# cv3vpl-lab/cylinder-pose-estimation

Hardware: AMD Instinct MI355X
Metric: frames/sec (grid-detect + cylinder fit) on 1920x1200 batch (higher is better)
Workload: dtype f64

## Files before the change

cylinder-pose-estimation_amd/csrc/ccl.hip:

```cpp
#include "cpe_dev.h"

namespace cpe {

namespace {

__device__ __forceinline__ bool pred(const uint8_t *img, size_t i, int thr, int invert)
{
    return (((int)img[i] > thr) ? 1 : 0) != invert;
}

constexpr int CCL_INIT_ROWS = 16;
__global__ __launch_bounds__(256) void k_ccl_init(const uint8_t *__restrict__ img, int rows_total, int h, int w,
                                                  int thr, int invert, const FrameState *__restrict__ st, Window win,
                                                  int *__restrict__ L, int *__restrict__ cnt, CclOutside outside)
{
    const int lane = threadIdx.x & 63;
    for (int rr = 0; rr < CCL_INIT_ROWS / 4; rr++) {
    const int row = (blockIdx.x * (CCL_INIT_ROWS / 4) + rr) * 4 + (threadIdx.x >> 6);
    if (row >= rows_total) return;
    const int f = row / h, y = row - f * h;
    const Rect r = window_rect(st, f, win, h, w);
    if (y < r.y0 || y > r.y1 || r.x1 < r.x0) continue;
    const size_t base = (size_t)row * w;
    int carry_in = 0, carry_start = 0;
// ... 876 lines not shown
static bool links8(const uint8_t *img, int n, int h, int w, int thr, Window win, int *L, FrameState *st, hipStream_t s)
{
    const size_t N = (size_t)h * w;
    if (word_rows(img, L, w)) {
        const ByteSrc src{img, w, thr, 0};
        CPE_KLAUNCH(k_ccl_init64<ByteSrc>, word_grid(n, h, w), dim3(256), 0, s, src, h, w, (const FrameState *)st, win, L);
        CPE_KLAUNCH(k_ccl_merge64<ByteSrc>, word_grid(n, h, w), dim3(256), 0, s, src, h, w, 1, (const FrameState *)st, win, L);
        return true;
    }
    CPE_KLAUNCH(k_ccl_init, dim3((n * h + CCL_INIT_ROWS - 1) / CCL_INIT_ROWS), dim3(256), 0, s, img, n * h, h, w, thr, 0, (const FrameState *)st, win, L,
                (int *)nullptr, OUTSIDE_UNTOUCHED);
    CPE_KLAUNCH(k_ccl_merge, dim3((unsigned)((N + CCL_BLK_PX - 1) / CCL_BLK_PX), n), dim3(256), 0, s, img, h, w, thr, 0, 1, (const FrameState *)st, win, L);
    return false;
}

int ccl_components(const uint8_t *img, const uint32_t *bits, int n, int h, int w, int thr, Window win, int *L, int *roots,
                   RootList list, FrameState *st, hipStream_t s)
{
    const size_t N = (size_t)h * w;
    const dim3 gw = word_grid(n, h, w);
    CPE_LAUNCH_BEGIN();
    CPE_KLAUNCH(k_ccl_ctl, dim3((n + 63) / 64), dim3(64), 0, s, st, (int *)nullptr, n, CTL_RESET_ROOTS, list);
    if (bits && w % 16 == 0 && ((size_t)L & 15) == 0) {
        const BitSrc src{bit_plane(bits, 0, h, w), bit_tile_cols(w), bit_plane_words(h, w)};
        CPE_KLAUNCH(k_ccl_init64<BitSrc>, gw, dim3(256), 0, s, src, h, w, (const FrameState *)st, win, L);
        CPE_KLAUNCH(k_ccl_merge64<BitSrc>, gw, dim3(256), 0, s, src, h, w, 1, (const FrameState *)st, win, L);
        CPE_KLAUNCH(k_ccl_roots64<BitSrc>, gw, dim3(256), 0, s, src, h, w, st, win, (const int *)L, roots, list);
    } else if (links8(img, n, h, w, thr, win, L, st, s)) {
        CPE_KLAUNCH(k_ccl_roots64<ByteSrc>, gw, dim3(256), 0, s, (ByteSrc{img, w, thr, 0}), h, w, st, win, (const int *)L, roots, list);
    } else {
        CPE_KLAUNCH(k_ccl_roots4, dim3((unsigned)((N + CCL_BLK_PX - 1) / CCL_BLK_PX), n), dim3(256), 0, s, img, h, w, thr, 0, st, win, (const int *)L,
                    roots, list);
    }
    CPE_CHECK_LAUNCH("ccl_components");
    return CPE_OK;
}

int ccl_unions(const uint8_t *mask, int n, int h, int w, Window win, int *L, FrameState *st, hipStream_t s)
// ... 61 lines not shown
```

cylinder-pose-estimation_amd/csrc/cpe_dev.h:

```cpp
#pragma once
#include "cpe_internal.h"

namespace cpe {

constexpr int MAXROOTS = 262144;
enum { SWL_DARK = 0, SWL_BRIGHT = 1, SWL_TRACE = 2 };
__host__ __device__ inline int sweep_pool(int h, int w, int which)
{
    const long long N = (long long)h * w;
    long long v = which == SWL_TRACE ? N / 8 : N / 2;
    const long long lo = which == SWL_TRACE ? (1 << 18) : (1 << 19);
    v = v < lo ? lo : (v > (1 << 23) ? (1 << 23) : v);
    return (int)((v + 255) / 256 * 256);
}
constexpr int MAXJ = CPE_MAXJ;
constexpr int MAXB = 32768;
constexpr int MAXG = 32768;
constexpr int MAXG_LDS = 1024;
constexpr int GCAP = 48;
constexpr int MAXV = 131072;
constexpr int MAXL = CPE_MAXL;
constexpr int MAXLP = CPE_MAXLP;
constexpr int MAXSEG = 2048;

// ... 50 lines not shown
    int *lohi, *hull;
};
struct RegionProbe {
    int identity;
    double *blobs; int blob_cap; int *n_blobs;
    float *kp; int kp_cap; int *n_kp;
};
inline unsigned frame_waves(int lists, int lo, int hi)
{
    const int v = 16384 / (lists > 0 ? lists : 1);
    return (unsigned)(v < lo ? lo : (v > hi ? hi : v));
}
struct RegionSide { hipStream_t s; hipEvent_t clahe_done, dark_done, traced, medians;
                    hipEvent_t joints_done = nullptr, spot_done = nullptr; };
struct MaskBuffers {
    uint8_t *binary, *hmask, *vmask, *joints_mask, *tmpA, *tmpB, *g19, *cm, *mc, *roi_h, *roi_v, *base_h, *base_v, *exp_h,
        *exp_v, *touch;
    int *lab, *roots, *jtmp, *joints, *verts;
    int *lab_p, *roots_p, *lab_s, *roots_s;
    int *lab_h, *lab_v;
    uint32_t *bits;
    unsigned long long *best, *best_s;
    unsigned long long *fl_j;
    uint32_t *jbits;
    SegRec *segs;
};

enum { OVF_ROOTS = 1, OVF_LINES = 2, OVF_TRACE = 4, OVF_JOINTS = 8, OVF_VERTS = 16, OVF_SEGS = 32, OVF_KERNEL = 64,
       OVF_EXPAND = 128, OVF_BLOBS = 256, OVF_DISTS = 512, OVF_GROUPS = 1024, OVF_SWEEP = 2048 };
__device__ __forceinline__ void set_overflow(FrameState &S, int bit) { atomicOr(&S.overflow, bit); }

// ... 226 lines not shown
    double d00 = (double)a00;
    if (fabs(d00) > 1.1920928955078125e-07) {
        double db1_2, db1_6;
        if (d00 > 0) { db1_2 = 0.5; db1_6 = 0.16666666666666666666666666666667; }
        else { db1_2 = -0.5; db1_6 = -0.16666666666666666666666666666667; }
        m00 = d00 * db1_2;
        m10 = (double)a10 * db1_6;
        m01 = (double)a01 * db1_6;
    }
}

int build_bitplanes(const uint8_t *img, int n, int h, int w, int thr0, int step, int nplanes, uint32_t *planes, hipStream_t s);

int ccl_components(const uint8_t *img, const uint32_t *bits, int n, int h, int w, int thr, Window win, int *L, int *roots,
                   RootList list, FrameState *st, hipStream_t s);
int ccl_unions(const uint8_t *mask, int n, int h, int w, Window win, int *L, FrameState *st, hipStream_t s);
int ccl_dark_first(const uint8_t *img, const uint32_t *planes, int nplanes, int n, int h, int w, int thr, int *L, int *roots,
                   int *cnt, FrameState *st, hipStream_t s);
enum CclOutside : int { OUTSIDE_NONE = 0, OUTSIDE_UNTOUCHED = 1, OUTSIDE_SWEEP_RUNS = 3 };
enum CclCount : int { COUNT_NONE = 0, COUNT_ALL = 1, COUNT_INTERIOR = 2, COUNT_ZERO = 3 };
struct CclPass {
    int thr = 0, invert = 0, conn8 = 1;
    Window win = WIN_FRAME;
    CclOutside outside = OUTSIDE_NONE;
    CclCount count = COUNT_NONE; int *cnt = nullptr;
    uint8_t *touch = nullptr;
    int *roots = nullptr;
    int *nrect = nullptr;
};
int ccl_label(const uint8_t *img, int n, int h, int w, int *L, const CclPass &p, FrameState *st, hipStream_t s);
// ... 29 lines not shown
```

cylinder-pose-estimation_amd/csrc/detect.hip:

```cpp
#include "workspace.h"
#include <ctype.h>
#include <mutex>
#include <stdlib.h>

namespace cpe {

namespace {

__global__ void k_state_init(FrameState *st, int n, unsigned long long *best, unsigned long long *best_s, int *nrect)
{
    int f = blockIdx.x * blockDim.x + threadIdx.x;
    if (f >= n) return;
    FrameState z = {};
    z.srect[0] = INT_MAX; z.srect[1] = INT_MAX; z.srect[2] = -1; z.srect[3] = -1;
    st[f] = z;
    if (best) { best[f] = 0; best_s[f] = 0; }
    if (nrect) { nrect[16 * f] = INT_MAX; nrect[16 * f + 1] = INT_MAX; nrect[16 * f + 2] = -1; nrect[16 * f + 3] = -1; }
}

__global__ void k_finish(const FrameState *st, int n, int *status, int *n_pts)
{
    int f = blockIdx.x * blockDim.x + threadIdx.x;
    if (f >= n) return;
    int s = st[f].status;
// ... 53 lines not shown
    R.lab = W.at<int>(WS_LABELS); R.cnt = W.at<int>(WS_LABELS_AUX); R.roots = W.at<int>(WS_ROOTS); R.nrect = W.at<int>(WS_NRECT);
    R.lab2 = W.at<int>(WS_BRIGHT_NODES); R.cnt2 = W.at<int>(WS_BRIGHT_COUNTS); R.sw = W.at<int>(WS_SWEEP); R.bk = W.at<int>(WS_BUCKET_PIXELS);
    R.hl = W.at<int2>(WS_LIST_DARK); R.bl = W.at<int2>(WS_LIST_BRIGHT); R.tl = W.at<int2>(WS_LIST_TRACE);
    R.bits = W.at<uint32_t>(WS_BITS); R.pool = W.at<uint32_t>(WS_POOL); R.blob_ch = W.at<unsigned short>(WS_BLOB_CH);
    R.maxch = region_maxch(h, w); R.maxdf = region_maxdf(h, w); R.gmid = W.at<double>(WS_GMID);
    R.hist = W.at<unsigned int>(WS_HIST); R.lut = W.at<uint8_t>(WS_LUT);
    R.blobs = W.at<BlobRec>(WS_BLOBS); R.blob_d = W.at<int>(WS_BLOB_D); R.order = W.at<int>(WS_ORDER); R.dists = W.at<double>(WS_DISTS);
    R.groups = W.at<Group>(WS_GROUPS); R.best = W.at<unsigned long long>(WS_BEST); R.lohi = W.at<int>(WS_LOHI); R.hull = W.at<int>(WS_HULL);
    return R;
}

MaskBuffers mask_buffers(const Workspace &W, const RegionBuffers &R)
{
    MaskBuffers M;
    M.binary = W.at<uint8_t>(WS_BINARY); M.hmask = W.at<uint8_t>(WS_HMASK); M.vmask = W.at<uint8_t>(WS_VMASK);
    M.joints_mask = W.at<uint8_t>(WS_JOINTS_MASK); M.tmpA = W.at<uint8_t>(WS_TMPA); M.tmpB = W.at<uint8_t>(WS_TMPB);
    M.g19 = W.at<uint8_t>(WS_BLUR19); M.cm = W.at<uint8_t>(WS_CM); M.mc = R.mc; M.roi_h = W.at<uint8_t>(WS_ROI_H);
    M.roi_v = W.at<uint8_t>(WS_ROI_V); M.base_h = W.at<uint8_t>(WS_BASE_H); M.base_v = W.at<uint8_t>(WS_BASE_V);
    M.exp_h = W.at<uint8_t>(WS_EXP_H); M.exp_v = W.at<uint8_t>(WS_EXP_V); M.touch = R.touch; M.bits = R.bits;
    M.lab = R.lab; M.roots = R.roots; M.jtmp = W.at<int>(WS_JTMP); M.joints = W.at<int>(WS_JOINTS); M.verts = W.at<int>(WS_VERTS);
    M.best = R.best; M.segs = W.at<SegRec>(WS_SEGS);
    M.lab_p = W.at<int>(WS_LABELS_JOINTS); M.lab_s = W.at<int>(WS_LABELS_SPOT);
    M.roots_p = W.at<int>(WS_ROOTS_JOINTS); M.roots_s = W.at<int>(WS_ROOTS_SPOT); M.best_s = W.at<unsigned long long>(WS_BEST_SPOT);
    M.fl_j = W.at<unsigned long long>(WS_FLJ); M.jbits = W.at<uint32_t>(WS_JOINT_BITS);
    M.lab_h = nullptr; M.lab_v = nullptr;
    return M;
}

}
}

// ... 460 lines not shown
```

cylinder-pose-estimation_amd/csrc/masks.hip:

```cpp
#include "cpe_dev.h"

namespace cpe {

namespace {

struct W3 { unsigned long long a, b, c; };
template <int K> __device__ __forceinline__ W3 w3_up(const W3 &v, unsigned long long fill)
{
    W3 r;
    r.a = (v.a >> K) | (v.b << (64 - K));
    r.b = (v.b >> K) | (v.c << (64 - K));
    r.c = (v.c >> K) | (fill << (64 - K));
    return r;
}
template <int K> __device__ __forceinline__ W3 w3_down(const W3 &v, unsigned long long fill)
{
    W3 r;
    r.c = (v.c << K) | (v.b >> (64 - K));
    r.b = (v.b << K) | (v.a >> (64 - K));
    r.a = (v.a << K) | (fill >> (64 - K));
    return r;
}
__device__ __forceinline__ W3 w3_and(const W3 &x, const W3 &y) { return W3{x.a & y.a, x.b & y.b, x.c & y.c}; }
__device__ __forceinline__ W3 w3_or(const W3 &x, const W3 &y) { return W3{x.a | y.a, x.b | y.b, x.c | y.c}; }
// ... 126 lines not shown
                    hm[o + b] = ((hb >> b) & 1u) ? 255 : 0;
                    vm[o + b] = ((vb >> b) & 1u) ? 255 : 0;
                    jm[o + b] = (((hb & vb) >> b) & 1u) ? 255 : 0;
                }
            }
        }
        store_plane_band(bit_plane(jbits, f, h, w), h, w, y0, R, t, [&](int tr, int j) {
            const size_t wi = (size_t)tr * WW + j;
            unsigned long long m = hbuf[wi] & (buf0[wi] | ((tr + 12 < ROWS) ? buf1[wi + (size_t)12 * WW] : 0ull));
            if (64 * j + 64 > w) m &= (1ull << (w - 64 * j)) - 1ull;
            return m;
        });
    }
}

__global__ __launch_bounds__(256) void k_or_and(const uint8_t *__restrict__ a, const uint8_t *__restrict__ b,
                                                const uint8_t *__restrict__ c, int h, int w, const FrameState *__restrict__ st,
                                                uint8_t *__restrict__ dst)
{
    const int N = h * w;
    const size_t f = blockIdx.y;
    const int *r = st[f].rect;
    const bool none = st[f].status == CPE_ST_NO_REGION;
    const int y0 = r[1], y1 = r[1] + r[3] - 1;
    const size_t o = f * (size_t)N;
    const bool vec = ((((size_t)a | (size_t)b | (size_t)c | (size_t)dst) & 15) == 0) && (N % 16 == 0);
    for (int it = 0; it < 4; it++) {
        const int i0 = blockIdx.x * 16384 + it * 4096 + threadIdx.x * 16;
        if (i0 >= N) break;
        const int ya = i0 / w, yb = min(i0 + 15, N - 1) / w;
        const bool outside = none || yb < y0 || ya > y1;
        if (vec) {
            uint4 v = make_uint4(0, 0, 0, 0);
            if (!outside) {
                const uint4 va = *reinterpret_cast<const uint4 *>(a + o + i0), vb = *reinterpret_cast<const uint4 *>(b + o + i0);
                const uint4 vc = *reinterpret_cast<const uint4 *>(c + o + i0);
                auto f4 = [](uint32_t x, uint32_t y, uint32_t z) {
                    uint32_t r4 = 0;
#pragma unroll
                    for (int k = 0; k < 4; k++) {
                        const uint32_t on = (((x | y) >> (8 * k)) & 255u) ? 255u : 0u;
                        r4 |= (on & ((z >> (8 * k)) & 255u)) << (8 * k);
                    }
                    return r4;
                };
                v = make_uint4(f4(va.x, vb.x, vc.x), f4(va.y, vb.y, vc.y), f4(va.z, vb.z, vc.z), f4(va.w, vb.w, vc.w));
            }
            *reinterpret_cast<uint4 *>(dst + o + i0) = v;
        } else {
            for (int k = 0; k < 16 && i0 + k < N; k++) {
                const size_t gi = o + i0 + k;
                dst[gi] = outside ? 0 : (uint8_t)(((a[gi] ? 255 : 0) | (b[gi] ? 255 : 0)) & c[gi]);
            }
        }
    }
}

constexpr int RB_R = 64, RB_AP = 4, RB_ROWS = RB_R + 2 * RB_AP;
__global__ __launch_bounds__(256) void k_roi_base(const uint8_t *__restrict__ m, const uint8_t *__restrict__ cm,
                                                  const uint8_t *__restrict__ mc, int h, int w, int bands,
                                                  const FrameState *__restrict__ st, uint8_t *__restrict__ roi,
                                                  uint8_t *__restrict__ base, uint32_t *__restrict__ bbits)
{
    extern __shared__ unsigned long long s_rb[];
    const int WW = (w + 63) >> 6;
    unsigned long long *buf0 = s_rb, *buf1 = s_rb + (size_t)RB_ROWS * WW;
    const int t = threadIdx.x;
    const int f = blockIdx.x / bands, band = blockIdx.x - f * bands;
    const int y0 = band * RB_R;
    const size_t N = (size_t)h * w;
    const int *rc = st[f].rect;
    const int rx0 = rc[0], ry0 = rc[1], rx1 = rc[0] + rc[2] - 1, ry1 = rc[1] + rc[3] - 1;
    const bool al8 = ((w & 7) == 0) && ((((size_t)m | (size_t)cm | (size_t)mc | (size_t)roi | (size_t)base) & 7) == 0);
    const int per_row = WW * 8;
    auto store8 = [&](uint8_t *dst, size_t o, int x0, unsigned bits) {
        if (al8) *reinterpret_cast<unsigned long long *>(dst + o) = bytes_of_bits8(bits);
        else for (int b = 0; b < 8 && x0 + b < w; b++) dst[o + b] = ((bits >> b) & 1u) ? 255 : 0;
    };
    if (st[f].status == CPE_ST_NO_REGION || y0 > ry1 + RB_AP || y0 + RB_R - 1 < ry0 - RB_AP) {
        for (int i = t; i < RB_R * per_row; i += 256) {
            const int tr = i / per_row, k = i - tr * per_row;
            const int y = y0 + tr, x0 = k * 8;
            if (y >= h || x0 >= w) continue;
            const size_t o = f * N + (size_t)y * w + x0;
            store8(roi, o, x0, 0u); store8(base, o, x0, 0u);
        }
        store_plane_band(bit_plane(bbits, f, h, w), h, w, y0, RB_R, t, [](int, int) { return 0ull; });
        return;
    }
    {
        uint8_t *pk = reinterpret_cast<uint8_t *>(buf0);
        for (int i = t; i < RB_ROWS * per_row; i += 256) {
            const int r = i / per_row, k = i - r * per_row;
            const int y = y0 - RB_AP + r, x0 = k * 8;
            unsigned bits = 0u;
            if (y >= ry0 && y <= ry1 && y >= 0 && y < h && x0 < w && x0 + 7 >= rx0 && x0 <= rx1) {
                const size_t o = f * N + (size_t)y * w + x0;
                if (al8) {
                    unsigned long long v = *reinterpret_cast<const unsigned long long *>(m + o) &
                                           *reinterpret_cast<const unsigned long long *>(cm + o) &
                                           *reinterpret_cast<const unsigned long long *>(mc + o);
                    v = (((v & 0x7f7f7f7f7f7f7f7full) + 0x7f7f7f7f7f7f7f7full) | v) & 0x8080808080808080ull;
                    bits = (unsigned)(((v >> 7) * 0x0102040810204080ull) >> 56);
                } else {
                    for (int b = 0; b < 8 && x0 + b < w; b++) bits |= ((m[o + b] & cm[o + b]) & mc[o + b]) ? (1u << b) : 0u;
                }
            }
            pk[i] = (uint8_t)bits;
        }
    }
    __syncthreads();
    auto pass = [&](const unsigned long long *src, unsigned long long *dst, bool dil) {
        const unsigned long long fill = dil ? 0ull : ~0ull;
        for (int i = t; i < RB_ROWS * WW; i += 256) {
            const int r = i / WW, j = i - r * WW;
            unsigned long long acc = fill;
#pragma unroll
            for (int dr = -1; dr <= 1; dr++) {
                const int rr = r + dr, y = y0 - RB_AP + rr;
                unsigned long long hres = fill;
                if (rr >= 0 && rr < RB_ROWS && y >= 0 && y < h) {
                    const unsigned long long *row = src + (size_t)rr * WW;
                    const unsigned long long va = row_valid_word(j - 1, w), vb = row_valid_word(j, w), vc = row_valid_word(j + 1, w);
                    unsigned long long xa = j > 0 ? row[j - 1] : 0ull, xb = row[j], xc = j + 1 < WW ? row[j + 1] : 0ull;
                    if (!dil) { xa |= ~va; xb |= ~vb; xc |= ~vc; }
                    const unsigned long long up = (xb >> 1) | (xc << 63), down = (xb << 1) | (xa >> 63);
                    hres = dil ? (xb | up | down) : (xb & up & down);
                }
                acc = dil ? (acc | hres) : (acc & hres);
            }
            const int y = y0 - RB_AP + r;
            dst[i] = (y >= 0 && y < h) ? (acc & row_valid_word(j, w)) : 0ull;
        }
        __syncthreads();
    };
    auto emit = [&](const unsigned long long *src, uint8_t *dst) {
        for (int i = t; i < RB_R * per_row; i += 256) {
            const int tr = i / per_row, k = i - tr * per_row;
            const int y = y0 + tr, x0 = k * 8;
            if (y >= h || x0 >= w) continue;
            const unsigned bits = (unsigned)(src[(size_t)(tr + RB_AP) * WW + (k >> 3)] >> ((k & 7) * 8)) & 255u;
            store8(dst, f * N + (size_t)y * w + x0, x0, bits);
        }
    };
    pass(buf0, buf1, false);
    pass(buf1, buf0, true);
    emit(buf0, roi);
    pass(buf0, buf1, true);
    pass(buf1, buf0, false);
    emit(buf0, base);
    store_plane_band(bit_plane(bbits, f, h, w), h, w, y0, RB_R, t, [&](int tr, int j) { return buf0[(size_t)(tr + RB_AP) * WW + j]; });
}

__global__ __launch_bounds__(64) void k_joint_centroids(const uint32_t *__restrict__ jbits, int h, int w,
                                                        const int *__restrict__ roots, FrameState *__restrict__ st,
                                                        int *__restrict__ jtmp ,
                                                        const unsigned long long *__restrict__ outside, size_t plane_words)
{
    __shared__ unsigned long long s_win[BW_ROWS * 64];
    const int f = blockIdx.y;
    if (st[f].status != CPE_ST_OK) return;
    const int ncomp = min(st[f].n_roots_p, MAXROOTS);
    for (int k = blockIdx.x * 64 + threadIdx.x; k < ncomp; k += gridDim.x * 64) {
        const int root = roots[(size_t)f * MAXROOTS + k];
        if (!comp_is_external(outside + f * plane_words, w, root, 0)) continue;
// ... 698 lines not shown
            rank += (aj < ai || (aj == ai && j < i)) ? 1 : 0;
        }
        if (rank == k_lo) s_lo = ai;
        if (rank == k_hi) s_hi = ai;
        atomicMax(&s_len, __float_as_uint(S[i].len));
    }
    __syncthreads();
    if (t == 0) {
        st[f].gang[which] = (nv & 1) ? s_hi : (float)(((double)s_lo + (double)s_hi) / 2.0);
        st[f].glen[which] = __uint_as_float(s_len);
    }
}

constexpr int EXP_MAXKS = 176;
constexpr int EXP_MAXKS_PLANE = 208;
template <int MAXKS>
__global__ __launch_bounds__(256) void k_seg_expand(const uint8_t *__restrict__ base, int h, int w, int which,
                                                    FrameState *__restrict__ st, const SegRec *__restrict__ segs,
                                                    uint8_t *__restrict__ exp, int fixed_ks)
{
    constexpr int EXP_REG = 15 + MAXKS + 2;
    __shared__ uint8_t dil[EXP_REG * EXP_REG];
    __shared__ short koff[4096][2];
    __shared__ short ppix[225][2];
    __shared__ int s_nk, s_np;
    const int f = blockIdx.y, t = threadIdx.x;
    FrameState &S = st[f];
    if (S.status != CPE_ST_OK) return;
    const int njobs = 2 * min(S.n_seg[which], MAXSEG);
    for (int job = blockIdx.x; job < njobs; job += gridDim.x) {
    const int seg = job >> 1, e = job & 1;
    const SegRec r = segs[(size_t)f * MAXSEG + seg];
    const float glen = S.glen[which], gang = S.gang[which];
    if ((double)r.len > 0.8 * (double)glen) continue;
    const int ks = fixed_ks > 0 ? fixed_ks : 91 + S.r0;
    if (ks > MAXKS) { if (t == 0) set_overflow(S, OVF_KERNEL); return; }
    __syncthreads();
    const float ak = fabsf(r.angle - gang) > 5.0f ? gang : r.angle;
    const int a = ks / 2, half = 7;
    const size_t N = (size_t)h * w;
    const uint8_t *bm = base + f * N;
    const int cx = (int)rint((double)(e ? r.p2x : r.p1x)), cy = (int)rint((double)(e ? r.p2y : r.p1y));
    const int x1 = max(cx - half, 0), x2 = min(cx + half + 1, w), y1 = max(cy - half, 0), y2 = min(cy + half + 1, h);
    if (t == 0) { s_nk = 0; s_np = 0; }
    __syncthreads();
    {
        const int c = ks / 2;
        double ar = (double)ak * 3.1415926535897932384626433832795 / 180.0;
        double alpha = cos(ar), beta = sin(ar);
        double M[6] = {alpha, beta, (1 - alpha) * c - beta * c, -beta, alpha, beta * c + (1 - alpha) * c};
        double D = M[0] * M[4] - M[1] * M[3];
        D = D != 0 ? 1. / D : 0;
        double A11 = M[4] * D, A22 = M[0] * D;
        double iM[6];
        iM[0] = A11; iM[1] = M[1] * (-D); iM[3] = M[3] * (-D); iM[4] = A22;
        double b1 = -iM[0] * M[2] - iM[1] * M[5];
        double b2 = -iM[3] * M[2] - iM[4] * M[5];
        iM[2] = b1; iM[5] = b2;
        for (int i = t; i < ks * ks; i += 256) {
            int y = i / ks, x = i - y * ks;
            int X0 = (int)rint((iM[1] * y + iM[2]) * 1024) + 512;
            int Y0 = (int)rint((iM[4] * y + iM[5]) * 1024) + 512;
            int adelta = (int)rint(iM[0] * x * 1024), bdelta = (int)rint(iM[3] * x * 1024);
            int X = (X0 + adelta) >> 10, Y = (Y0 + bdelta) >> 10;
            if (X >= 0 && X < ks && Y == c) {
                int q = atomicAdd(&s_nk, 1);
                if (q < 4096) { koff[q][0] = (short)(x - a); koff[q][1] = (short)(y - a); }
            }
        }
    }
    for (int i = t; i < 225; i += 256) {
        int py = y1 + i / 15, px = x1 + i % 15;
        if (py < y2 && px < x2 && bm[(size_t)py * w + px]) {
            int q = atomicAdd(&s_np, 1);
            ppix[q][0] = (short)px; ppix[q][1] = (short)py;
        }
    }
    const int bx1 = x1 - a - 1, by1 = y1 - a - 1;
    const int bw = (x2 - x1) + 2 * a + 2, bh = (y2 - y1) + 2 * a + 2;
    for (int i = t; i < bw * bh; i += 256) dil[i] = 0;
    __syncthreads();
    const int nk = min(s_nk, 4096), np = s_np;
    if (s_nk > 4096 && t == 0) set_overflow(S, OVF_EXPAND);
    for (int i = t; i < nk * np; i += 256) {
        int p = i / nk, k = i - p * nk;
        int xx = ppix[p][0] - koff[k][0], yy = ppix[p][1] - koff[k][1];
        if (xx >= 0 && xx < w && yy >= 0 && yy < h) dil[(yy - by1) * bw + (xx - bx1)] = 1;
    }
    __syncthreads();
    uint8_t *ex = exp + f * N;
    for (int i = t; i < bw * bh; i += 256) {
        int ly = i / bw, lx = i - ly * bw;
        int gy = by1 + ly, gx = bx1 + lx;
        if (gx < 0 || gx >= w || gy < 0 || gy >= h) continue;
        bool all = true;
        for (int dy = -1; dy <= 1 && all; dy++)
            for (int dx = -1; dx <= 1; dx++) {
                int yy = gy + dy, xx = gx + dx;
                if (yy < 0 || yy >= h || xx < 0 || xx >= w) continue;
                int ly2 = ly + dy, lx2 = lx + dx;
                bool v = (ly2 >= 0 && ly2 < bh && lx2 >= 0 && lx2 < bw) ? dil[ly2 * bw + lx2] != 0 : false;
                if (!v) { all = false; break; }
            }
        if (all) ex[(size_t)gy * w + gx] = 255;
    }
    }
}

__global__ void k_masks_reset(FrameState *st, int n)
{
    int f = blockIdx.x * blockDim.x + threadIdx.x;
    if (f >= n) return;
    FrameState &S = st[f];
    S.n_joints = 0; S.n_joints_all = 0; S.n_seg[0] = 0; S.n_seg[1] = 0;
    S.gang[0] = S.gang[1] = 0; S.glen[0] = S.glen[1] = 0;
    if (S.status == CPE_ST_NO_REGION) { S.r0 = 0; S.spot[0] = S.spot[1] = S.spot[2] = S.spot[3] = 0; }
    else if (S.status == CPE_ST_OK && S.spot_fail) S.status = CPE_ST_NO_SPOT;
}

// ... 121 lines not shown
        CPE_KLAUNCH(k_spot_scan, dim3((unsigned)(n * tiles_y)), dim3(256), 0, s, gray, h, w, tiles_x, tiles_y, st, flags, fstride);
        CPE_KLAUNCH(k_blur19_spot, dim3((unsigned)(n * tiles_y)), dim3(256), 0, s, gray, h, w, tiles_x, tiles_y, t19,
                    (const uint8_t *)flags, fstride, B.g19);
    }
    if ((rc = ccl_components(B.g19, nullptr, n, h, w, 240, WIN_SPOT, B.lab_s, B.roots_s, ROOTS_SPOT, st, s)) != CPE_OK) return rc;
    CPE_KLAUNCH(k_spot_area, dim3(4, n), dim3(64), 0, s, B.g19, h, w, B.roots_s, st, B.best_s);
    (void)hipMemsetAsync(B.cm, 255, total, s);
    CPE_KLAUNCH(k_spot_ellipse, dim3(n), dim3(64), 0, s, B.g19, n, h, w, B.best_s, st, B.verts, B.cm, planar);
    CPE_CHECK_LAUNCH("spot_stage");
    return CPE_OK;
}

int masks_stage(const uint8_t *gray, int n, int h, int w, const MaskBuffers &B, FrameState *st, hipStream_t s,
                const RegionSide *side, int planar, hipStream_t sj)
{
    const size_t total = (size_t)h * w * n;
    int rc;
    CPE_LAUNCH_BEGIN();
    CPE_KLAUNCH(k_masks_reset, dim3((n + 63) / 64), dim3(64), 0, s, st, n);
    const size_t fl_words = bit_plane_words(h, w);
    auto fl_plane = [&](int k) { return bit_plane(B.bits, (size_t)(2 + k) * n, h, w); };
    const bool jside = side && sj != s;
    if (jside) { (void)hipEventRecord(side->clahe_done, s); (void)hipStreamWaitEvent(sj, side->clahe_done, 0); }
    {
        hipStream_t q = jside ? sj : s;
        CPE_KLAUNCH(k_joint_centroids, dim3(frame_waves(n, 16, MAXROOTS / 64), n), dim3(64), 0, q, (const uint32_t *)B.jbits, h, w, B.roots_p, st, B.jtmp,
                    (const unsigned long long *)(B.fl_j + (size_t)n * h * ((w + 63) / 64)), (size_t)h * ((w + 63) / 64));
        CPE_KLAUNCH(k_joint_sort, dim3(n), dim3(256), 0, q, st, B.jtmp, B.joints);
    }
    const int rb_bands = (h + RB_R - 1) / RB_R;
    const size_t rb_lds = (size_t)2 * RB_ROWS * ((w + 63) / 64) * 8;
    CPE_CHECK_ARG(rb_lds <= 160 * 1024, "masks_stage: frame too wide (%d columns)", w);
    CPE_CHECK_HIP(hipFuncSetAttribute(reinterpret_cast<const void *>(&k_roi_base), hipFuncAttributeMaxDynamicSharedMemorySize, 160 * 1024));
    if (side) { (void)hipEventRecord(side->clahe_done, s); (void)hipStreamWaitEvent(side->s, side->clahe_done, 0); }
    for (int which = 0; which < 2; which++) {
        hipStream_t q = (which && side) ? side->s : s;
        const uint8_t *lm = which ? B.vmask : B.hmask;
        uint8_t *roi = which ? B.roi_v : B.roi_h;
        uint8_t *base = which ? B.base_v : B.base_h;
        uint8_t *exp = which ? B.exp_v : B.exp_h;
        uint8_t *tmp = which ? B.tmpA : B.tmpB;
        int *lab = which ? B.lab_s : B.lab, *roots = which ? B.roots_s : B.roots;
        const RootList list = which ? ROOTS_SPOT : ROOTS_MAIN;
        uint32_t *bits = reinterpret_cast<uint32_t *>(bit_plane(B.bits, which ? (size_t)n : 0, h, w));
        SegRec *segs = B.segs + (size_t)which * n * MAXSEG;
        CPE_KLAUNCH(k_roi_base, dim3((unsigned)(n * rb_bands)), dim3(256), rb_lds, q, lm, (const uint8_t *)B.cm, (const uint8_t *)B.mc,
                    h, w, rb_bands, (const FrameState *)st, roi, base, bits);
        if ((rc = ccl_components(base, bits, n, h, w, 0, WIN_REGION, lab, roots, list, st, q)) != CPE_OK) return rc;
        unsigned long long *fl_bg = fl_plane(2 + 2 * which), *fl_out = fl_plane(3 + 2 * which);
        if ((rc = outside_flood(base, n, h, w, st, WIN_REGION, fl_bg, fl_out, fl_words, q, bits)) != CPE_OK) return rc;
        if (planar) CPE_KLAUNCH((k_seg_trace<8, 700>), dim3(frame_waves(n, 32, 512), n), dim3(64), 0, q, (const uint32_t *)bits, h, w, which, (const int *)roots, list, st, segs, (const unsigned long long *)fl_out, fl_words);
        else CPE_KLAUNCH((k_seg_trace<5, 200>), dim3(frame_waves(n, 32, 512), n), dim3(64), 0, q, (const uint32_t *)bits, h, w, which, (const int *)roots, list, st, segs, (const unsigned long long *)fl_out, fl_words);
        CPE_KLAUNCH(k_seg_global, dim3(n), dim3(256), 0, q, st, which, (const SegRec *)segs);
        (void)hipMemsetAsync(tmp, 0, total, q);
        if (planar) CPE_KLAUNCH(k_seg_expand<EXP_MAXKS_PLANE>, dim3(frame_waves(n, 32, 256), n), dim3(256), 0, q, (const uint8_t *)base, h, w, which, st, (const SegRec *)segs, tmp, 201);
        else CPE_KLAUNCH(k_seg_expand<EXP_MAXKS>, dim3(frame_waves(n, 32, 256), n), dim3(256), 0, q, (const uint8_t *)base, h, w, which, st, (const SegRec *)segs, tmp, 0);
        CPE_KLAUNCH(k_or_and, dim3((unsigned)(((size_t)h * w + 16383) / 16384), n), dim3(256), 0, q, (const uint8_t *)tmp, (const uint8_t *)base,
                    (const uint8_t *)B.mc, h, w, (const FrameState *)st, exp);
        CPE_CHECK_LAUNCH("masks_stage expand");
        if ((rc = ccl_unions(exp, n, h, w, WIN_REGION, which ? B.lab_v : B.lab_h, st, q)) != CPE_OK) return rc;
    }
    if (side) { (void)hipEventRecord(side->traced, side->s); (void)hipStreamWaitEvent(s, side->traced, 0); }
    return CPE_OK;
}

}
```

cylinder-pose-estimation_amd/csrc/workspace.h:

```cpp
#pragma once
#include "cpe_dev.h"
#include <algorithm>
#include <string.h>

namespace cpe {
namespace {

enum WsOverlay {
    OV_NONE = 0,
    OV_BORDERS,
    OV_BRIGHT,
    OV_CHAINS,
    OV_DARK,
    OV_COUNT
};

static int region_maxch(int h, int w) { long long v = (long long)h * w / 256; return (int)std::min(65535LL, std::max(8192LL, v)); }
static int region_maxdf(int h, int w) { long long v = (long long)h * w / 16; return (int)std::max(65536LL, v); }

#define CPE_WS_TABLE(X) \
    X(DISTS,  (size_t)17 * region_maxdf(h, w) * sizeof(double), -1, OV_BORDERS, 0)    \
    X(POOL,   (size_t)17 * region_maxch(h, w) * 128,            -1, OV_BORDERS, 0)    \
    X(GROUPS, (size_t)MAXG * sizeof(Group),                     -1, OV_BORDERS, 1)    \
    X(BRIGHT_NODES,  N * 8, -1, OV_BRIGHT, 0)    \
    X(BRIGHT_COUNTS, N * 4, -1, OV_BRIGHT, 0)    \
    X(ROI_H,  N, CPE_PLANE_ROI_H, OV_BRIGHT, 1) \
    X(ROI_V,  N, CPE_PLANE_ROI_V, OV_BRIGHT, 1) \
    X(BASE_H, N, -1, OV_BRIGHT, 1) \
    X(BASE_V, N, -1, OV_BRIGHT, 1) \
    X(EXP_H,  N, CPE_PLANE_EXP_H, OV_BRIGHT, 1) \
    X(EXP_V,  N, CPE_PLANE_EXP_V, OV_BRIGHT, 1) \
    X(TMPA,   N, -1, OV_BRIGHT, 1) \
    X(TMPB,   N, -1, OV_BRIGHT, 1) \
    X(DISCS,  N, -1, OV_BRIGHT, 1)               \
    X(MASK_CONTOUR, N, CPE_PLANE_MASK_CONTOUR, OV_BRIGHT, 1) \
    X(BLUR7,  N, CPE_PLANE_BLUR7, OV_BRIGHT, 1) \
    X(LABELS_JOINTS, N * 4, -1, OV_CHAINS, 0)    \
    X(LABELS_SPOT,   N * 4, -1, OV_CHAINS, 0)    \
    X(LINES,  lines_ws_bytes(), -1, OV_CHAINS, 1)    \
    X(SUBPIX, (size_t)2 * MAXL * 2 * (size_t)(std::max(h, w) + 128) * sizeof(float), -1, OV_CHAINS, 1) \
    X(BLOB_CH, (size_t)17 * MAXB * 16 * sizeof(unsigned short), -1, OV_CHAINS, 2)    \
    X(BLOB_D,  (size_t)17 * MAXB * 2 * sizeof(int),             -1, OV_CHAINS, 2)    \
    X(LABELS,     N * 4, CPE_PLANE_LABELS, OV_DARK, 0)    \
    X(LABELS_AUX, N * 4, -1, OV_DARK, 0)         \
    X(BLOBS,  (size_t)17 * MAXB * sizeof(BlobRec), -1, OV_DARK, 1)    \
    X(BINARY, N, CPE_PLANE_BINARY, OV_NONE, 0) \
    X(HMASK,  N, CPE_PLANE_HMASK, OV_NONE, 0) \
    X(VMASK,  N, CPE_PLANE_VMASK, OV_NONE, 0) \
// ... 130 lines not shown
```

Baseline: 3610.

## Fuse segment-end expansion with base mask and drop tmp planes and or-and pass

k_roi_base now writes the base AND mc result directly into the exp plane and skips the byte base plane when CCL can read the bit plane. k_seg_expand reads base pixels from the bit plane, dilates with bitwise word rows and atomicOr, erodes with shifted word masks, and ORs results straight into exp under mc. Both segment ends are handled in one block, sharing the kernel-offset table. This removes the full-frame tmp memset, the k_or_and pass and one byte-plane write, at the cost of more LDS in k_roi_base and extra bit manipulation in expand.

```diff
diff --git a/cylinder-pose-estimation_amd/csrc/ccl.hip b/cylinder-pose-estimation_amd/csrc/ccl.hip
--- a/cylinder-pose-estimation_amd/csrc/ccl.hip
+++ b/cylinder-pose-estimation_amd/csrc/ccl.hip
@@ -914,6 +914,8 @@
     return false;
 }
 
+bool ccl_components_reads_bits(const uint32_t *bits, int w, const int *L) { return bits && w % 16 == 0 && ((size_t)L & 15) == 0; }
+
 int ccl_components(const uint8_t *img, const uint32_t *bits, int n, int h, int w, int thr, Window win, int *L, int *roots,
                    RootList list, FrameState *st, hipStream_t s)
 {
@@ -921,7 +923,7 @@
     const dim3 gw = word_grid(n, h, w);
     CPE_LAUNCH_BEGIN();
     CPE_KLAUNCH(k_ccl_ctl, dim3((n + 63) / 64), dim3(64), 0, s, st, (int *)nullptr, n, CTL_RESET_ROOTS, list);
-    if (bits && w % 16 == 0 && ((size_t)L & 15) == 0) {
+    if (ccl_components_reads_bits(bits, w, L)) {
         const BitSrc src{bit_plane(bits, 0, h, w), bit_tile_cols(w), bit_plane_words(h, w)};
         CPE_KLAUNCH(k_ccl_init64<BitSrc>, gw, dim3(256), 0, s, src, h, w, (const FrameState *)st, win, L);
         CPE_KLAUNCH(k_ccl_merge64<BitSrc>, gw, dim3(256), 0, s, src, h, w, 1, (const FrameState *)st, win, L);
diff --git a/cylinder-pose-estimation_amd/csrc/cpe_dev.h b/cylinder-pose-estimation_amd/csrc/cpe_dev.h
--- a/cylinder-pose-estimation_amd/csrc/cpe_dev.h
+++ b/cylinder-pose-estimation_amd/csrc/cpe_dev.h
@@ -88,7 +88,7 @@
 struct RegionSide { hipStream_t s; hipEvent_t clahe_done, dark_done, traced, medians;
                     hipEvent_t joints_done = nullptr, spot_done = nullptr; };
 struct MaskBuffers {
-    uint8_t *binary, *hmask, *vmask, *joints_mask, *tmpA, *tmpB, *g19, *cm, *mc, *roi_h, *roi_v, *base_h, *base_v, *exp_h,
+    uint8_t *binary, *hmask, *vmask, *joints_mask, *g19, *cm, *mc, *roi_h, *roi_v, *base_h, *base_v, *exp_h,
         *exp_v, *touch;
     int *lab, *roots, *jtmp, *joints, *verts;
     int *lab_p, *roots_p, *lab_s, *roots_s;
@@ -345,6 +345,7 @@
 
 int ccl_components(const uint8_t *img, const uint32_t *bits, int n, int h, int w, int thr, Window win, int *L, int *roots,
                    RootList list, FrameState *st, hipStream_t s);
+bool ccl_components_reads_bits(const uint32_t *bits, int w, const int *L);
 int ccl_unions(const uint8_t *mask, int n, int h, int w, Window win, int *L, FrameState *st, hipStream_t s);
 int ccl_dark_first(const uint8_t *img, const uint32_t *planes, int nplanes, int n, int h, int w, int thr, int *L, int *roots,
                    int *cnt, FrameState *st, hipStream_t s);
diff --git a/cylinder-pose-estimation_amd/csrc/detect.hip b/cylinder-pose-estimation_amd/csrc/detect.hip
--- a/cylinder-pose-estimation_amd/csrc/detect.hip
+++ b/cylinder-pose-estimation_amd/csrc/detect.hip
@@ -91,7 +91,7 @@
 {
     MaskBuffers M;
     M.binary = W.at<uint8_t>(WS_BINARY); M.hmask = W.at<uint8_t>(WS_HMASK); M.vmask = W.at<uint8_t>(WS_VMASK);
-    M.joints_mask = W.at<uint8_t>(WS_JOINTS_MASK); M.tmpA = W.at<uint8_t>(WS_TMPA); M.tmpB = W.at<uint8_t>(WS_TMPB);
+    M.joints_mask = W.at<uint8_t>(WS_JOINTS_MASK);
     M.g19 = W.at<uint8_t>(WS_BLUR19); M.cm = W.at<uint8_t>(WS_CM); M.mc = R.mc; M.roi_h = W.at<uint8_t>(WS_ROI_H);
     M.roi_v = W.at<uint8_t>(WS_ROI_V); M.base_h = W.at<uint8_t>(WS_BASE_H); M.base_v = W.at<uint8_t>(WS_BASE_V);
     M.exp_h = W.at<uint8_t>(WS_EXP_H); M.exp_v = W.at<uint8_t>(WS_EXP_V); M.touch = R.touch; M.bits = R.bits;
diff --git a/cylinder-pose-estimation_amd/csrc/masks.hip b/cylinder-pose-estimation_amd/csrc/masks.hip
--- a/cylinder-pose-estimation_amd/csrc/masks.hip
+++ b/cylinder-pose-estimation_amd/csrc/masks.hip
@@ -164,64 +164,23 @@
     }
 }
 
-__global__ __launch_bounds__(256) void k_or_and(const uint8_t *__restrict__ a, const uint8_t *__restrict__ b,
-                                                const uint8_t *__restrict__ c, int h, int w, const FrameState *__restrict__ st,
-                                                uint8_t *__restrict__ dst)
-{
-    const int N = h * w;
-    const size_t f = blockIdx.y;
-    const int *r = st[f].rect;
-    const bool none = st[f].status == CPE_ST_NO_REGION;
-    const int y0 = r[1], y1 = r[1] + r[3] - 1;
-    const size_t o = f * (size_t)N;
-    const bool vec = ((((size_t)a | (size_t)b | (size_t)c | (size_t)dst) & 15) == 0) && (N % 16 == 0);
-    for (int it = 0; it < 4; it++) {
-        const int i0 = blockIdx.x * 16384 + it * 4096 + threadIdx.x * 16;
-        if (i0 >= N) break;
-        const int ya = i0 / w, yb = min(i0 + 15, N - 1) / w;
-        const bool outside = none || yb < y0 || ya > y1;
-        if (vec) {
-            uint4 v = make_uint4(0, 0, 0, 0);
-            if (!outside) {
-                const uint4 va = *reinterpret_cast<const uint4 *>(a + o + i0), vb = *reinterpret_cast<const uint4 *>(b + o + i0);
-                const uint4 vc = *reinterpret_cast<const uint4 *>(c + o + i0);
-                auto f4 = [](uint32_t x, uint32_t y, uint32_t z) {
-                    uint32_t r4 = 0;
-#pragma unroll
-                    for (int k = 0; k < 4; k++) {
-                        const uint32_t on = (((x | y) >> (8 * k)) & 255u) ? 255u : 0u;
-                        r4 |= (on & ((z >> (8 * k)) & 255u)) << (8 * k);
-                    }
-                    return r4;
-                };
-                v = make_uint4(f4(va.x, vb.x, vc.x), f4(va.y, vb.y, vc.y), f4(va.z, vb.z, vc.z), f4(va.w, vb.w, vc.w));
-            }
-            *reinterpret_cast<uint4 *>(dst + o + i0) = v;
-        } else {
-            for (int k = 0; k < 16 && i0 + k < N; k++) {
-                const size_t gi = o + i0 + k;
-                dst[gi] = outside ? 0 : (uint8_t)(((a[gi] ? 255 : 0) | (b[gi] ? 255 : 0)) & c[gi]);
-            }
-        }
-    }
-}
-
 constexpr int RB_R = 64, RB_AP = 4, RB_ROWS = RB_R + 2 * RB_AP;
 __global__ __launch_bounds__(256) void k_roi_base(const uint8_t *__restrict__ m, const uint8_t *__restrict__ cm,
                                                   const uint8_t *__restrict__ mc, int h, int w, int bands,
                                                   const FrameState *__restrict__ st, uint8_t *__restrict__ roi,
-                                                  uint8_t *__restrict__ base, uint32_t *__restrict__ bbits)
+                                                  uint8_t *__restrict__ base, uint8_t *__restrict__ exp,
+                                                  uint32_t *__restrict__ bbits)
 {
     extern __shared__ unsigned long long s_rb[];
     const int WW = (w + 63) >> 6;
-    unsigned long long *buf0 = s_rb, *buf1 = s_rb + (size_t)RB_ROWS * WW;
+    unsigned long long *buf0 = s_rb, *buf1 = s_rb + (size_t)RB_ROWS * WW, *mcb = s_rb + (size_t)2 * RB_ROWS * WW;
     const int t = threadIdx.x;
     const int f = blockIdx.x / bands, band = blockIdx.x - f * bands;
     const int y0 = band * RB_R;
     const size_t N = (size_t)h * w;
     const int *rc = st[f].rect;
     const int rx0 = rc[0], ry0 = rc[1], rx1 = rc[0] + rc[2] - 1, ry1 = rc[1] + rc[3] - 1;
-    const bool al8 = ((w & 7) == 0) && ((((size_t)m | (size_t)cm | (size_t)mc | (size_t)roi | (size_t)base) & 7) == 0);
+    const bool al8 = ((w & 7) == 0) && ((((size_t)m | (size_t)cm | (size_t)mc | (size_t)roi | (size_t)base | (size_t)exp) & 7) == 0);
     const int per_row = WW * 8;
     auto store8 = [&](uint8_t *dst, size_t o, int x0, unsigned bits) {
         if (al8) *reinterpret_cast<unsigned long long *>(dst + o) = bytes_of_bits8(bits);
@@ -233,30 +192,38 @@
             const int y = y0 + tr, x0 = k * 8;
             if (y >= h || x0 >= w) continue;
             const size_t o = f * N + (size_t)y * w + x0;
-            store8(roi, o, x0, 0u); store8(base, o, x0, 0u);
+            store8(roi, o, x0, 0u); store8(exp, o, x0, 0u);
+            if (base) store8(base, o, x0, 0u);
         }
         store_plane_band(bit_plane(bbits, f, h, w), h, w, y0, RB_R, t, [](int, int) { return 0ull; });
         return;
     }
     {
-        uint8_t *pk = reinterpret_cast<uint8_t *>(buf0);
+        uint8_t *pk = reinterpret_cast<uint8_t *>(buf0), *pkc = reinterpret_cast<uint8_t *>(mcb);
+        auto nonzero8 = [](unsigned long long v) {
+            v = (((v & 0x7f7f7f7f7f7f7f7full) + 0x7f7f7f7f7f7f7f7full) | v) & 0x8080808080808080ull;
+            return (unsigned)(((v >> 7) * 0x0102040810204080ull) >> 56);
+        };
         for (int i = t; i < RB_ROWS * per_row; i += 256) {
             const int r = i / per_row, k = i - r * per_row;
             const int y = y0 - RB_AP + r, x0 = k * 8;
-            unsigned bits = 0u;
+            unsigned bits = 0u, cbits = 0u;
             if (y >= ry0 && y <= ry1 && y >= 0 && y < h && x0 < w && x0 + 7 >= rx0 && x0 <= rx1) {
                 const size_t o = f * N + (size_t)y * w + x0;
                 if (al8) {
-                    unsigned long long v = *reinterpret_cast<const unsigned long long *>(m + o) &
-                                           *reinterpret_cast<const unsigned long long *>(cm + o) &
-                                           *reinterpret_cast<const unsigned long long *>(mc + o);
-                    v = (((v & 0x7f7f7f7f7f7f7f7full) + 0x7f7f7f7f7f7f7f7full) | v) & 0x8080808080808080ull;
-                    bits = (unsigned)(((v >> 7) * 0x0102040810204080ull) >> 56);
+                    const unsigned long long vc = *reinterpret_cast<const unsigned long long *>(mc + o);
+                    bits = nonzero8(*reinterpret_cast<const unsigned long long *>(m + o) &
+                                    *reinterpret_cast<const unsigned long long *>(cm + o) & vc);
+                    cbits = nonzero8(vc);
                 } else {
-                    for (int b = 0; b < 8 && x0 + b < w; b++) bits |= ((m[o + b] & cm[o + b]) & mc[o + b]) ? (1u << b) : 0u;
+                    for (int b = 0; b < 8 && x0 + b < w; b++) {
+                        bits |= ((m[o + b] & cm[o + b]) & mc[o + b]) ? (1u << b) : 0u;
+                        cbits |= mc[o + b] ? (1u << b) : 0u;
+                    }
                 }
             }
             pk[i] = (uint8_t)bits;
+            pkc[i] = (uint8_t)cbits;
         }
     }
     __syncthreads();
@@ -284,21 +251,24 @@
         }
         __syncthreads();
     };
-    auto emit = [&](const unsigned long long *src, uint8_t *dst) {
+    auto emit = [&](const unsigned long long *src, uint8_t *dst, uint8_t *dst2, const unsigned long long *and2) {
         for (int i = t; i < RB_R * per_row; i += 256) {
             const int tr = i / per_row, k = i - tr * per_row;
             const int y = y0 + tr, x0 = k * 8;
             if (y >= h || x0 >= w) continue;
-            const unsigned bits = (unsigned)(src[(size_t)(tr + RB_AP) * WW + (k >> 3)] >> ((k & 7) * 8)) & 255u;
-            store8(dst, f * N + (size_t)y * w + x0, x0, bits);
+            const size_t wi = (size_t)(tr + RB_AP) * WW + (k >> 3);
+            const unsigned bits = (unsigned)(src[wi] >> ((k & 7) * 8)) & 255u;
+            const size_t o = f * N + (size_t)y * w + x0;
+            if (dst) store8(dst, o, x0, bits);
+            if (dst2) store8(dst2, o, x0, bits & (unsigned)(and2[wi] >> ((k & 7) * 8)));
         }
     };
     pass(buf0, buf1, false);
     pass(buf1, buf0, true);
-    emit(buf0, roi);
+    emit(buf0, roi, nullptr, nullptr);
     pass(buf0, buf1, true);
     pass(buf1, buf0, false);
-    emit(buf0, base);
+    emit(buf0, base, exp, mcb);
     store_plane_band(bit_plane(bbits, f, h, w), h, w, y0, RB_R, t, [&](int tr, int j) { return buf0[(size_t)(tr + RB_AP) * WW + j]; });
 }
 
@@ -1027,22 +997,30 @@
 
 constexpr int EXP_MAXKS = 176;
 constexpr int EXP_MAXKS_PLANE = 208;
+constexpr int EXP_NT = 256, EXP_WW = 4, EXP_MAXOFF = 4096;
 template <int MAXKS>
-__global__ __launch_bounds__(256) void k_seg_expand(const uint8_t *__restrict__ base, int h, int w, int which,
-                                                    FrameState *__restrict__ st, const SegRec *__restrict__ segs,
-                                                    uint8_t *__restrict__ exp, int fixed_ks)
+__global__ __launch_bounds__(EXP_NT) void k_seg_expand(const uint32_t *__restrict__ base_bits, const uint8_t *__restrict__ mc, int h, int w,
+                                                       int which, FrameState *__restrict__ st, const SegRec *__restrict__ segs,
+                                                       uint8_t *__restrict__ exp, int fixed_ks)
 {
     constexpr int EXP_REG = 15 + MAXKS + 2;
-    __shared__ uint8_t dil[EXP_REG * EXP_REG];
-    __shared__ short koff[4096][2];
-    __shared__ short ppix[225][2];
-    __shared__ int s_nk, s_np;
+    static_assert(EXP_REG <= 64 * EXP_WW, "a support row must fit EXP_WW words");
+    __shared__ unsigned long long dil[EXP_REG * EXP_WW];
+    __shared__ short koff[EXP_MAXOFF][2];
+    __shared__ int tX0[MAXKS], tY0[MAXKS], tA[MAXKS], tB[MAXKS];
+    __shared__ unsigned long long vc[EXP_WW];
+    __shared__ unsigned prow[15];
+    __shared__ int s_nk;
     const int f = blockIdx.y, t = threadIdx.x;
     FrameState &S = st[f];
     if (S.status != CPE_ST_OK) return;
-    const int njobs = 2 * min(S.n_seg[which], MAXSEG);
-    for (int job = blockIdx.x; job < njobs; job += gridDim.x) {
-    const int seg = job >> 1, e = job & 1;
+    const int nseg = min(S.n_seg[which], MAXSEG);
+    const size_t N = (size_t)h * w;
+    const unsigned long long *bp = bit_plane(base_bits, f, h, w);
+    const int btc = bit_tile_cols(w);
+    const uint8_t *mcf = mc + f * N;
+    uint8_t *ex = exp + f * N;
+    for (int seg = blockIdx.x; seg < nseg; seg += gridDim.x) {
     const SegRec r = segs[(size_t)f * MAXSEG + seg];
     const float glen = S.glen[which], gang = S.gang[which];
     if ((double)r.len > 0.8 * (double)glen) continue;
@@ -1051,14 +1029,9 @@
     __syncthreads();
     const float ak = fabsf(r.angle - gang) > 5.0f ? gang : r.angle;
     const int a = ks / 2, half = 7;
-    const size_t N = (size_t)h * w;
-    const uint8_t *bm = base + f * N;
-    const int cx = (int)rint((double)(e ? r.p2x : r.p1x)), cy = (int)rint((double)(e ? r.p2y : r.p1y));
-    const int x1 = max(cx - half, 0), x2 = min(cx + half + 1, w), y1 = max(cy - half, 0), y2 = min(cy + half + 1, h);
-    if (t == 0) { s_nk = 0; s_np = 0; }
-    __syncthreads();
+    if (t == 0) s_nk = 0;
+    const int c = ks / 2;
     {
-        const int c = ks / 2;
         double ar = (double)ak * 3.1415926535897932384626433832795 / 180.0;
         double alpha = cos(ar), beta = sin(ar);
         double M[6] = {alpha, beta, (1 - alpha) * c - beta * c, -beta, alpha, beta * c + (1 - alpha) * c};
@@ -1070,52 +1043,92 @@
         double b1 = -iM[0] * M[2] - iM[1] * M[5];
         double b2 = -iM[3] * M[2] - iM[4] * M[5];
         iM[2] = b1; iM[5] = b2;
-        for (int i = t; i < ks * ks; i += 256) {
-            int y = i / ks, x = i - y * ks;
-            int X0 = (int)rint((iM[1] * y + iM[2]) * 1024) + 512;
-            int Y0 = (int)rint((iM[4] * y + iM[5]) * 1024) + 512;
-            int adelta = (int)rint(iM[0] * x * 1024), bdelta = (int)rint(iM[3] * x * 1024);
-            int X = (X0 + adelta) >> 10, Y = (Y0 + bdelta) >> 10;
+        for (int i = t; i < ks; i += EXP_NT) {
+            tX0[i] = (int)rint((iM[1] * i + iM[2]) * 1024) + 512;
+            tY0[i] = (int)rint((iM[4] * i + iM[5]) * 1024) + 512;
+            tA[i] = (int)rint(iM[0] * i * 1024);
+            tB[i] = (int)rint(iM[3] * i * 1024);
+        }
+    }
+    __syncthreads();
+    for (int y = t >> 6; y < ks; y += EXP_NT / 64) {
+        const int X0 = tX0[y], Y0 = tY0[y];
+        for (int x = t & 63; x < ks; x += 64) {
+            const int X = (X0 + tA[x]) >> 10, Y = (Y0 + tB[x]) >> 10;
             if (X >= 0 && X < ks && Y == c) {
                 int q = atomicAdd(&s_nk, 1);
-                if (q < 4096) { koff[q][0] = (short)(x - a); koff[q][1] = (short)(y - a); }
+                if (q < EXP_MAXOFF) { koff[q][0] = (short)(x - a); koff[q][1] = (short)(y - a); }
             }
         }
     }
-    for (int i = t; i < 225; i += 256) {
-        int py = y1 + i / 15, px = x1 + i % 15;
-        if (py < y2 && px < x2 && bm[(size_t)py * w + px]) {
-            int q = atomicAdd(&s_np, 1);
-            ppix[q][0] = (short)px; ppix[q][1] = (short)py;
-        }
-    }
+    __syncthreads();
+    const int nk = min(s_nk, EXP_MAXOFF);
+    if (s_nk > EXP_MAXOFF && t == 0) set_overflow(S, OVF_EXPAND);
+    for (int e = 0; e < 2; e++) {
+    const int cx = (int)rint((double)(e ? r.p2x : r.p1x)), cy = (int)rint((double)(e ? r.p2y : r.p1y));
+    const int x1 = max(cx - half, 0), x2 = min(cx + half + 1, w), y1 = max(cy - half, 0), y2 = min(cy + half + 1, h);
+    if (x2 <= x1 || y2 <= y1) continue;
     const int bx1 = x1 - a - 1, by1 = y1 - a - 1;
-    const int bw = (x2 - x1) + 2 * a + 2, bh = (y2 - y1) + 2 * a + 2;
-    for (int i = t; i < bw * bh; i += 256) dil[i] = 0;
-    __syncthreads();
-    const int nk = min(s_nk, 4096), np = s_np;
-    if (s_nk > 4096 && t == 0) set_overflow(S, OVF_EXPAND);
-    for (int i = t; i < nk * np; i += 256) {
-        int p = i / nk, k = i - p * nk;
-        int xx = ppix[p][0] - koff[k][0], yy = ppix[p][1] - koff[k][1];
-        if (xx >= 0 && xx < w && yy >= 0 && yy < h) dil[(yy - by1) * bw + (xx - bx1)] = 1;
-    }
-    __syncthreads();
-    uint8_t *ex = exp + f * N;
-    for (int i = t; i < bw * bh; i += 256) {
-        int ly = i / bw, lx = i - ly * bw;
-        int gy = by1 + ly, gx = bx1 + lx;
-        if (gx < 0 || gx >= w || gy < 0 || gy >= h) continue;
-        bool all = true;
-        for (int dy = -1; dy <= 1 && all; dy++)
-            for (int dx = -1; dx <= 1; dx++) {
-                int yy = gy + dy, xx = gx + dx;
-                if (yy < 0 || yy >= h || xx < 0 || xx >= w) continue;
-                int ly2 = ly + dy, lx2 = lx + dx;
-                bool v = (ly2 >= 0 && ly2 < bh && lx2 >= 0 && lx2 < bw) ? dil[ly2 * bw + lx2] != 0 : false;
-                if (!v) { all = false; break; }
-            }
-        if (all) ex[(size_t)gy * w + gx] = 255;
+    const int bh = (y2 - y1) + 2 * a + 2;
+    if (e) __syncthreads();
+    for (int i = t; i < bh * EXP_WW; i += EXP_NT) dil[i] = 0ull;
+    if (t < 15) {
+        const int y = y1 + t;
+        unsigned m = 0u;
+        if (y < y2) {
+            const int j = x1 >> 6, sh = x1 & 63;
+            unsigned long long v = bp[bit_word(btc, y, j)] >> sh;
+            if (sh) v |= bp[bit_word(btc, y, j + 1)] << (64 - sh);
+            m = (unsigned)v & ((1u << (x2 - x1)) - 1u);
+        }
+        prow[t] = m;
+    } else if (t >= 16 && t < 16 + EXP_WW) {
+        const int wd = t - 16;
+        const int lo = min(max(-bx1 - 64 * wd, 0), 64), hi = min(max(w - bx1 - 64 * wd, 0), 64);
+        unsigned long long v = 0ull;
+        if (hi > lo) v = (hi == 64 ? ~0ull : ((1ull << hi) - 1ull)) & ~((1ull << lo) - 1ull);
+        vc[wd] = v;
+    }
+    __syncthreads();
+    for (int i = t; i < nk * 15; i += EXP_NT) {
+        const int k = i / 15, pr = i - k * 15;
+        const unsigned long long m = prow[pr];
+        const int yy = y1 + pr - koff[k][1];
+        if (!m || yy < 0 || yy >= h) continue;
+        const int sh = a + 1 - koff[k][0];
+        const int wd = sh >> 6, b = sh & 63;
+        unsigned long long *row = dil + (yy - by1) * EXP_WW;
+        const unsigned long long lo = (m << b) & vc[wd];
+        if (lo) atomicOr(&row[wd], lo);
+        if (b > 49) {
+            const unsigned long long hi = (m >> (64 - b)) & vc[wd + 1];
+            if (hi) atomicOr(&row[wd + 1], hi);
+        }
+    }
+    __syncthreads();
+    for (int i = t; i < (bh - 2) * EXP_WW * 4; i += EXP_NT) {
+        const int ly = 1 + (i >> 4), wd = (i >> 2) & 3, off = (i & 3) * 16;
+        const int gy = by1 + ly;
+        if (gy < 0 || gy >= h || !((dil[ly * EXP_WW + wd] >> off) & 0xffffull)) continue;
+        unsigned long long acc = vc[wd];
+#pragma unroll
+        for (int dr = -1; dr <= 1; dr++) {
+            if (gy + dr < 0 || gy + dr >= h) continue;
+            const unsigned long long *row = dil + (ly + dr) * EXP_WW;
+            const unsigned long long xb = row[wd] | ~vc[wd];
+            const unsigned long long xa = wd > 0 ? (row[wd - 1] | ~vc[wd - 1]) : 0ull;
+            const unsigned long long xc = wd + 1 < EXP_WW ? (row[wd + 1] | ~vc[wd + 1]) : 0ull;
+            acc &= xb & ((xb >> 1) | (xc << 63)) & ((xb << 1) | (xa >> 63));
+        }
+        unsigned bits = (unsigned)(acc >> off) & 0xffffu;
+        const size_t o = (size_t)gy * w + (bx1 + wd * 64 + off);
+        while (bits) {
+            const int b = __ffs(bits) - 1;
+            bits &= bits - 1u;
+            const uint8_t cv = mcf[o + b];
+            if (cv) ex[o + b] = 255 & cv;
+        }
+    }
     }
     }
 }
@@ -1267,7 +1280,6 @@
 int masks_stage(const uint8_t *gray, int n, int h, int w, const MaskBuffers &B, FrameState *st, hipStream_t s,
                 const RegionSide *side, int planar, hipStream_t sj)
 {
-    const size_t total = (size_t)h * w * n;
     int rc;
     CPE_LAUNCH_BEGIN();
     CPE_KLAUNCH(k_masks_reset, dim3((n + 63) / 64), dim3(64), 0, s, st, n);
@@ -1282,7 +1294,7 @@
         CPE_KLAUNCH(k_joint_sort, dim3(n), dim3(256), 0, q, st, B.jtmp, B.joints);
     }
     const int rb_bands = (h + RB_R - 1) / RB_R;
-    const size_t rb_lds = (size_t)2 * RB_ROWS * ((w + 63) / 64) * 8;
+    const size_t rb_lds = (size_t)3 * RB_ROWS * ((w + 63) / 64) * 8;
     CPE_CHECK_ARG(rb_lds <= 160 * 1024, "masks_stage: frame too wide (%d columns)", w);
     CPE_CHECK_HIP(hipFuncSetAttribute(reinterpret_cast<const void *>(&k_roi_base), hipFuncAttributeMaxDynamicSharedMemorySize, 160 * 1024));
     if (side) { (void)hipEventRecord(side->clahe_done, s); (void)hipStreamWaitEvent(side->s, side->clahe_done, 0); }
@@ -1290,26 +1302,22 @@
         hipStream_t q = (which && side) ? side->s : s;
         const uint8_t *lm = which ? B.vmask : B.hmask;
         uint8_t *roi = which ? B.roi_v : B.roi_h;
-        uint8_t *base = which ? B.base_v : B.base_h;
         uint8_t *exp = which ? B.exp_v : B.exp_h;
-        uint8_t *tmp = which ? B.tmpA : B.tmpB;
         int *lab = which ? B.lab_s : B.lab, *roots = which ? B.roots_s : B.roots;
         const RootList list = which ? ROOTS_SPOT : ROOTS_MAIN;
         uint32_t *bits = reinterpret_cast<uint32_t *>(bit_plane(B.bits, which ? (size_t)n : 0, h, w));
         SegRec *segs = B.segs + (size_t)which * n * MAXSEG;
+        uint8_t *base = ccl_components_reads_bits(bits, w, lab) ? nullptr : (which ? B.base_v : B.base_h);
         CPE_KLAUNCH(k_roi_base, dim3((unsigned)(n * rb_bands)), dim3(256), rb_lds, q, lm, (const uint8_t *)B.cm, (const uint8_t *)B.mc,
-                    h, w, rb_bands, (const FrameState *)st, roi, base, bits);
+                    h, w, rb_bands, (const FrameState *)st, roi, base, exp, bits);
         if ((rc = ccl_components(base, bits, n, h, w, 0, WIN_REGION, lab, roots, list, st, q)) != CPE_OK) return rc;
         unsigned long long *fl_bg = fl_plane(2 + 2 * which), *fl_out = fl_plane(3 + 2 * which);
         if ((rc = outside_flood(base, n, h, w, st, WIN_REGION, fl_bg, fl_out, fl_words, q, bits)) != CPE_OK) return rc;
         if (planar) CPE_KLAUNCH((k_seg_trace<8, 700>), dim3(frame_waves(n, 32, 512), n), dim3(64), 0, q, (const uint32_t *)bits, h, w, which, (const int *)roots, list, st, segs, (const unsigned long long *)fl_out, fl_words);
         else CPE_KLAUNCH((k_seg_trace<5, 200>), dim3(frame_waves(n, 32, 512), n), dim3(64), 0, q, (const uint32_t *)bits, h, w, which, (const int *)roots, list, st, segs, (const unsigned long long *)fl_out, fl_words);
         CPE_KLAUNCH(k_seg_global, dim3(n), dim3(256), 0, q, st, which, (const SegRec *)segs);
-        (void)hipMemsetAsync(tmp, 0, total, q);
-        if (planar) CPE_KLAUNCH(k_seg_expand<EXP_MAXKS_PLANE>, dim3(frame_waves(n, 32, 256), n), dim3(256), 0, q, (const uint8_t *)base, h, w, which, st, (const SegRec *)segs, tmp, 201);
-        else CPE_KLAUNCH(k_seg_expand<EXP_MAXKS>, dim3(frame_waves(n, 32, 256), n), dim3(256), 0, q, (const uint8_t *)base, h, w, which, st, (const SegRec *)segs, tmp, 0);
-        CPE_KLAUNCH(k_or_and, dim3((unsigned)(((size_t)h * w + 16383) / 16384), n), dim3(256), 0, q, (const uint8_t *)tmp, (const uint8_t *)base,
-                    (const uint8_t *)B.mc, h, w, (const FrameState *)st, exp);
+        if (planar) CPE_KLAUNCH(k_seg_expand<EXP_MAXKS_PLANE>, dim3(frame_waves(n, 32, 256), n), dim3(EXP_NT), 0, q, (const uint32_t *)bits, (const uint8_t *)B.mc, h, w, which, st, (const SegRec *)segs, exp, 201);
+        else CPE_KLAUNCH(k_seg_expand<EXP_MAXKS>, dim3(frame_waves(n, 32, 256), n), dim3(EXP_NT), 0, q, (const uint32_t *)bits, (const uint8_t *)B.mc, h, w, which, st, (const SegRec *)segs, exp, 0);
         CPE_CHECK_LAUNCH("masks_stage expand");
         if ((rc = ccl_unions(exp, n, h, w, WIN_REGION, which ? B.lab_v : B.lab_h, st, q)) != CPE_OK) return rc;
     }
diff --git a/cylinder-pose-estimation_amd/csrc/workspace.h b/cylinder-pose-estimation_amd/csrc/workspace.h
--- a/cylinder-pose-estimation_amd/csrc/workspace.h
+++ b/cylinder-pose-estimation_amd/csrc/workspace.h
@@ -26,12 +26,12 @@
     X(BRIGHT_COUNTS, N * 4, -1, OV_BRIGHT, 0)    \
     X(ROI_H,  N, CPE_PLANE_ROI_H, OV_BRIGHT, 1) \
     X(ROI_V,  N, CPE_PLANE_ROI_V, OV_BRIGHT, 1) \
-    X(BASE_H, N, -1, OV_BRIGHT, 1) \
+    X(BASE_H, N, -1, OV_BRIGHT, 1)               \
     X(BASE_V, N, -1, OV_BRIGHT, 1) \
     X(EXP_H,  N, CPE_PLANE_EXP_H, OV_BRIGHT, 1) \
     X(EXP_V,  N, CPE_PLANE_EXP_V, OV_BRIGHT, 1) \
-    X(TMPA,   N, -1, OV_BRIGHT, 1) \
-    X(TMPB,   N, -1, OV_BRIGHT, 1) \
+    X(TMPA,   N, -1, OV_BRIGHT, 1)               \
+    X(TMPB,   N, -1, OV_BRIGHT, 1)               \
     X(DISCS,  N, -1, OV_BRIGHT, 1)               \
     X(MASK_CONTOUR, N, CPE_PLANE_MASK_CONTOUR, OV_BRIGHT, 1) \
     X(BLUR7,  N, CPE_PLANE_BLUR7, OV_BRIGHT, 1) \
```

New measurement: 3725, median of 6. 1.03x the previous value.
